# bempt/uda_aerial_semantic_segmentation_research

Hardware: AMD Instinct MI355X
Metric: training images/sec at 512x512 (higher is better)
Workload: dtype fp32

## Files before the change

### include/udaseg.h

```cpp
#ifndef UDASEG_H
#define UDASEG_H

#include <stddef.h>
#include <stdint.h>

#ifdef __cplusplus
extern "C" {
#endif

#define UDASEG_OK 0
#define UDASEG_E_BADARG (-1)
#define UDASEG_E_UNSUPPORTED (-2)
#define UDASEG_E_WORKSPACE (-3)
#define UDASEG_E_HIP (-4)

#define UDASEG_ACT_NONE 0
#define UDASEG_ACT_LEAKY 1

int udaseg_version(void);
#define UDASEG_OPT_GENERIC_GATHER 0
#define UDASEG_OPT_F32_SPLIT 1
#define UDASEG_OPT_WGRAD_GENERIC 2
#define UDASEG_OPT_F32_HALO 3
#define UDASEG_OPT_F3_CFG 4
// ... 5 lines not shown
#define UDASEG_OPT_WGRAD_X3_BLOCKS 10
#define UDASEG_OPT_WGRAD_BLOCKS 11
#define UDASEG_OPT_WGRAD_NO_XCD 12
#define UDASEG_OPT_WGRAD_X3 13
#define UDASEG_OPT_NO_WGRAD_HALO 14
#define UDASEG_OPT_WGRAD_F3_BLOCKS 15
#define UDASEG_OPT_WGRAD_HALO_BLOCKS 16
#define UDASEG_OPT_WGRAD_DEEP_BLOCKS 17
#define UDASEG_OPT_WGRAD_DB 18
#define UDASEG_OPT_REDUCE_BLOCKS 19
#define UDASEG_OPT_BN_APPLY_PT 20
#define UDASEG_OPT_GEMM_1X1_TILE 21
#define UDASEG_OPT_GEMM_1X1 22
#define UDASEG_OPT_GEMM_1X1_MAXM 23
#define UDASEG_OPT_NO_STREAM 24
#define UDASEG_OPT_HALO_CFG 25
#define UDASEG_OPT_NO_HALO 26
#define UDASEG_OPT_NO_HALO_S2 27
#define UDASEG_OPT_HALO_W16 28
#define UDASEG_OPT_HALO_DEEP 29
#define UDASEG_OPT_HALO_S2_CK 30
#define UDASEG_OPT_UP_CFG 31
#define UDASEG_OPT_WGRAD_UP_BLOCKS 32
#define UDASEG_OPT_COUNT 33
int udaseg_set_option(int key, int value);
int udaseg_get_option(int key);
int udaseg_option_count(void);
const char* udaseg_option_name(int key);
int udaseg_option_epoch(void);
const char* udaseg_last_error(void);
int udaseg_device_count(void);
int udaseg_memset_async(void* ptr, int value, size_t bytes, void* stream);
int udaseg_stream_wait(void* waiter_stream, void* signal_stream);

typedef struct {
  int n, hi, wi, ci;
  int ho, wo, co;
  int kh, kw, stride, pad;
} udaseg_conv_desc;


int udaseg_conv2d_fwd(const udaseg_conv_desc* d, const float* x, const float* w, const float* bias, float* y,
                      int act, float slope, int accumulate, void* stream);
int udaseg_conv2d_fwd_bnstats(const udaseg_conv_desc* d, const float* x, const float* w, const float* bias, float* y,
                              double* stats, void* stream);
int udaseg_conv2d_fwd_fused(const udaseg_conv_desc* d, const float* x, const float* w, const float* bias,
                            const float* residual, float* y, int act, float slope, void* stream);
// ... 328 lines not shown
```

### uda_aerial_semantic_segmentation_research_amd/_lib.py

```python
import ctypes as C
import os

_HERE = os.path.dirname(os.path.abspath(__file__))
LIB_PATH = os.environ.get("UDASEG_LIB", os.path.join(_HERE, "libudaseg_hip.so"))

ACT_NONE = 0
ACT_LEAKY = 1


class ConvDesc(C.Structure):
    _fields_ = [(k, C.c_int) for k in ("n", "hi", "wi", "ci", "ho", "wo", "co", "kh", "kw", "stride", "pad")]


_P = C.c_void_p
_I = C.c_int
_L = C.c_int64
_F = C.c_float
_D = C.POINTER(ConvDesc)

SIGNATURES = {
    "udaseg_version": (_I, []),
    "udaseg_set_option": (_I, [_I, _I]),
    "udaseg_get_option": (_I, [_I]),
    "udaseg_option_count": (_I, []),
# ... 145 lines not shown
    "udaseg_conv2d_wgrad_up_f32x3": (_I, [_D, _P, _I, _P, _P, _P]),
    "udaseg_conv2d_wgrad_halo_slice_f32x3": (_I, [_D, _P, _P, _P, _I, _I, _P]),
    "udaseg_wgrad_up_set_blocks": (_I, [_I]),
    "udaseg_conv_stem_f32x3_ok": (_I, [_D]),
    "udaseg_conv2d_fwd_stem_f32x3": (_I, [_D, _P, _P, _P, _P, _P]),
    "udaseg_conv_n16_f32x3_ok": (_I, [_D, _I]),
    "udaseg_conv2d_fwd_n16_f32x3": (_I, [_D, _P, _P, _P, _I, _F, _P, _P, _P, _P]),
    "udaseg_conv2d_dgrad_n16_f32x3": (_I, [_D, _P, _P, _P, _P, _P, _P, _P, _P, _I, _F, _P, _P]),
    "udaseg_set_workspace": (_I, [_P, C.c_size_t]),
    "udaseg_workspace_bytes": (C.c_size_t, [_D]),
    "udaseg_debug_set_timeline": (_I, [_P, _I]),
    "udaseg_fill_f32": (_I, [_P, _L, _F, _P]),
    "udaseg_axpy_f32": (_I, [_P, _P, _L, _F, _P]),
    "udaseg_add_i64": (_I, [_P, _L, _L, _P]),
    "udaseg_prof_enable": (_I, [_I]),
    "udaseg_prof_reset": (_I, []),
    "udaseg_prof_read": (_I, [_I, C.POINTER(C.c_double), C.POINTER(C.c_double), C.POINTER(C.c_int64)]),
    "udaseg_prof_kernel_count": (_I, []),
    "udaseg_prof_kernel_name": (C.c_char_p, [_I]),
    "udaseg_prof_kernel_read": (_I, [_I, C.POINTER(C.c_double), C.POINTER(C.c_double), C.POINTER(C.c_int64)]),
    "udaseg_prof_records": (_I, [_I, _I, C.POINTER(C.c_double), C.POINTER(C.c_double), C.POINTER(C.c_int), C.POINTER(C.c_int)]),
}

OPTIONS = {"GENERIC_GATHER": 0, "F32_SPLIT": 1, "WGRAD_GENERIC": 2, "F32_HALO": 3, "F3_CFG": 4, "F3_WS": 5, "F3_SIGNS": 6, "IGEMM_TILE": 7, "IGEMM_X3": 8, "NO_FOLD": 9, "WGRAD_X3_BLOCKS": 10, "WGRAD_BLOCKS": 11, "WGRAD_NO_XCD": 12, "WGRAD_X3": 13, "NO_WGRAD_HALO": 14, "WGRAD_F3_BLOCKS": 15, "WGRAD_HALO_BLOCKS": 16, "WGRAD_DEEP_BLOCKS": 17, "WGRAD_DB": 18, "REDUCE_BLOCKS": 19, "BN_APPLY_PT": 20, "GEMM_1X1_TILE": 21, "GEMM_1X1": 22, "GEMM_1X1_MAXM": 23, "NO_STREAM": 24, "HALO_CFG": 25, "NO_HALO": 26, "NO_HALO_S2": 27, "HALO_W16": 28, "HALO_DEEP": 29, "HALO_S2_CK": 30, "UP_CFG": 31, "WGRAD_UP_BLOCKS": 32}

_lib = None


def load():
    global _lib
    if _lib is not None:
        return _lib
    if not os.path.exists(LIB_PATH):
        raise RuntimeError(
            f"{LIB_PATH} not found: the HIP extension is not built. Run `python -c \"import __graft_entry__ as g; "
            f"g.build()\"` (or `make -C {os.path.join(_HERE, 'csrc')}`). There is no CPU fallback.")
    lib = C.CDLL(LIB_PATH)
    for name, (res, args) in SIGNATURES.items():
        fn = getattr(lib, name)
        fn.restype = res
        fn.argtypes = args
    _lib = lib
    return lib


def check(rc, what=""):
    if rc != 0:
# ... 10 lines not shown
```

### uda_aerial_semantic_segmentation_research_amd/csrc/api.hip

```cpp
#include <string.h>
#include <mutex>
#include <vector>

#include "common.h"
#include "options.h"

namespace udaseg {

static thread_local char g_err[512] = "";

void set_error(const char* fmt, ...) {
  va_list ap;
  va_start(ap, fmt);
  vsnprintf(g_err, sizeof(g_err), fmt, ap);
  va_end(ap);
}

int hip_fail(hipError_t e, const char* what) {
  set_error("%s: %s", what, hipGetErrorString(e));
  return UDASEG_E_HIP;
}

struct ProfRec {
  hipEvent_t a, b;
// ... 221 lines not shown
     {"UDASEG_NO_FOLD", K_FLAG, 0},
     {"UDASEG_WGRAD_X3_BLOCKS", K_INT, 1024},
     {"UDASEG_WGRAD_BLOCKS", K_INT, 0},
     {"UDASEG_WGRAD_NO_XCD", K_FLAG, 0},
     {"UDASEG_WGRAD_X3", K_OFF0, 1},
     {"UDASEG_NO_WGRAD_HALO", K_FLAG, 0},
     {"UDASEG_WGRAD_F3_BLOCKS", K_INT, 120},
     {"UDASEG_WGRAD_HALO_BLOCKS", K_INT, 96},
     {"UDASEG_WGRAD_DEEP_BLOCKS", K_INT, 0},
     {"UDASEG_WGRAD_DB", K_INT, 1},
     {"UDASEG_REDUCE_BLOCKS", K_INT, 0},
     {"UDASEG_BN_APPLY_PT", K_INT, 4},
     {"UDASEG_GEMM_1X1_TILE", K_INT, 0},
     {"UDASEG_GEMM_1X1", K_OFF0, 1},
     {"UDASEG_GEMM_1X1_MAXM", K_INT, 73728},
     {"UDASEG_NO_STREAM", K_FLAG, 0},
     {"UDASEG_HALO_CFG", K_INT, 0},
     {"UDASEG_NO_HALO", K_FLAG, 0},
     {"UDASEG_NO_HALO_S2", K_FLAG, 0},
     {"UDASEG_HALO_W16", K_INT, 6},
     {"UDASEG_HALO_DEEP", K_OFF0, 1},
     {"UDASEG_HALO_S2_CK", K_INT, 64},
     {"UDASEG_UP_CFG", K_INT, 0},
     {"UDASEG_WGRAD_UP_BLOCKS", K_INT, 0}};
int g_opt_val[UDASEG_OPT_COUNT];
static int g_opt_default[UDASEG_OPT_COUNT];
std::atomic<bool> g_opt_ready{false};
static std::atomic<int> g_opt_epoch{0};
static std::mutex g_opt_mutex;
void opt_init() {
  std::lock_guard<std::mutex> lk(g_opt_mutex);
  if (g_opt_ready.load(std::memory_order_relaxed)) return;
  for (int k = 0; k < UDASEG_OPT_COUNT; ++k) {
    const OptRow& r = g_opt_rows[k];
    const char* e = getenv(r.env);
    int v = r.dflt;
    if (r.kind == K_INT) v = e ? atoi(e) : r.dflt;
    else if (r.kind == K_FLAG) v = e != nullptr ? 1 : 0;
    else v = (e && atoi(e) == 0) ? 0 : 1;
    g_opt_default[k] = g_opt_val[k] = v;
  }
  g_opt_ready.store(true, std::memory_order_release);
}
}

extern "C" int udaseg_set_option(int key, int value) {
  UDASEG_CHECK_ARG(key >= 0 && key < UDASEG_OPT_COUNT, "set_option: unknown key %d (0 .. %d)", key, UDASEG_OPT_COUNT - 1);
// ... 40 lines not shown
```

### uda_aerial_semantic_segmentation_research_amd/csrc/conv_wgrad.hip

```cpp
#include <stdlib.h>

#include <type_traits>

#include "common.h"
#include "halo_common.h"

namespace udaseg {

struct WgradArgs {
  const void* x;
  const void* dy;
  float* dw;
  int hi, wi, ci, ho, wo, co;
  int kw, stride, pad;
  int M, J;
  int kchunk;
  int use_atomic;
  float inv_ci, inv_kw, inv_wo, inv_ho;
  int row_uniform;
  unsigned x_bytes, dy_bytes;
  int ci_full, c_off, J_ld, up;
  const float* in_scale;
  const float* in_shift;
  int in_act;
// ... 953 lines not shown
  return f32 ? (off || !f32_halo_enabled()) : off;
}
}

extern "C" int udaseg_conv2d_wgrad_bnin_ok(const udaseg_conv_desc* d, int up) {
  if (!d || d->kh != 3 || d->kw != 3 || d->stride != 1 || d->pad != 1 || d->n <= 0 || d->hi <= 0 || d->wi <= 0 || d->ci % 8 != 0 ||
      d->co % 4 != 0)
    return 0;
  if (small_wgrad_applicable(d->kh, d->stride, d->pad, d->ci, d->co, d->n * cdiv(d->hi, 16) * cdiv(d->wi, 16))) return 1;
  return !up && !wgrad_halo_off(true) && wgrad_h2_applicable(d, 0, true) ? 1 : 0;
}

extern "C" int udaseg_conv2d_wgrad_bnin(const udaseg_conv_desc* d, const float* x, int up, const float* in_scale, const float* in_shift,
                                        int in_act, float in_slope, const float* dy, float* dw, int accumulate, void* stream) {
  UDASEG_CHECK_ARG(d && x && in_scale && in_shift && dy && dw, "conv2d_wgrad_bnin: NULL pointer");
  UDASEG_CHECK_ARG(in_act == UDASEG_ACT_NONE || in_act == UDASEG_ACT_LEAKY, "conv2d_wgrad_bnin: unknown activation %d", in_act);
  UDASEG_CHECK_ARG(d->ho == d->hi && d->wo == d->wi, "conv2d_wgrad_bnin: stride-1 'same' convolutions only");
  UDASEG_CHECK_ARG(!up || (d->hi % 2 == 0 && d->wi % 2 == 0), "conv2d_wgrad_bnin: an up-sampled source needs even extents");
  if (!udaseg_conv2d_wgrad_bnin_ok(d, up)) {
    set_error("conv2d_wgrad_bnin: geometry not supported (ask udaseg_conv2d_wgrad_bnin_ok)");
    return UDASEG_E_UNSUPPORTED;
  }
  hipStream_t st = as_stream(stream);
  const bool small = small_wgrad_applicable(d->kh, d->stride, d->pad, d->ci, d->co, d->n * cdiv(d->hi, 16) * cdiv(d->wi, 16));
  if (!small && !accumulate) {
    hipError_t e = hipMemsetAsync(dw, 0, (size_t)d->co * 9 * d->ci * sizeof(float), st);
    if (e != hipSuccess) return hip_fail(e, "hipMemsetAsync(dw)");
  }
  prof_begin(1, st);
  int rc;
  if (small) {
    rc = launch_small_wgrad(x, dy, dw, d->n, d->hi, d->wi, d->ci, d->co, accumulate, st, up, in_scale, in_shift, in_act, in_slope);
  } else {
    rc = launch_wgrad_h2(d, x, nullptr, 0, dy, dw, true, st, in_scale, in_shift, in_act, in_slope);
  }
  prof_end(1, st, udaseg_conv_flops(d), 2, d);
  return rc;
}

extern "C" int udaseg_conv2d_wgrad_halo_bf16_ok(const udaseg_conv_desc* d, int up_ca) {
  return d != nullptr && !wgrad_halo_off(false) && wgrad_h2_applicable(d, up_ca, false) ? 1 : 0;
}

extern "C" int udaseg_conv2d_wgrad_halo_bf16(const udaseg_conv_desc* d, const void* x, const void* skip, int up_ca, const void* dy,
                                             float* dw, void* stream) {
  UDASEG_CHECK_ARG(d && x && dy && dw, "conv2d_wgrad_halo_bf16: NULL pointer");
  UDASEG_CHECK_ARG(d->n > 0 && d->hi > 0 && d->wi > 0 && d->ho == d->hi && d->wo == d->wi, "conv2d_wgrad_halo_bf16: bad extents");
  UDASEG_CHECK_ARG(up_ca == 0 ? skip == nullptr : skip != nullptr, "conv2d_wgrad_halo_bf16: up_ca and skip come together");
  if (!udaseg_conv2d_wgrad_halo_bf16_ok(d, up_ca)) {
    set_error("conv2d_wgrad_halo_bf16: geometry not supported (ask udaseg_conv2d_wgrad_halo_bf16_ok first)");
    return UDASEG_E_UNSUPPORTED;
  }
  hipStream_t st = as_stream(stream);
  prof_begin(1, st);
  const int rc = launch_wgrad_h2(d, x, skip, up_ca, dy, dw, false, st);
  prof_end(1, st, udaseg_conv_flops(d), 2, d);
  return rc;
}

extern "C" int udaseg_conv2d_wgrad_halo_f32x3_ok(const udaseg_conv_desc* d, int up_ca) {
  return d != nullptr && !wgrad_halo_off(true) && wgrad_h2_applicable(d, up_ca, true) ? 1 : 0;
}

extern "C" int udaseg_conv2d_wgrad_halo_f32x3(const udaseg_conv_desc* d, const float* x, const float* skip, int up_ca, const float* dy,
                                              float* dw, void* stream) {
  UDASEG_CHECK_ARG(d && x && dy && dw, "conv2d_wgrad_halo_f32x3: NULL pointer");
  UDASEG_CHECK_ARG(d->n > 0 && d->hi > 0 && d->wi > 0 && d->ho == d->hi && d->wo == d->wi, "conv2d_wgrad_halo_f32x3: bad extents");
  UDASEG_CHECK_ARG((up_ca > 0) == (skip != nullptr), "conv2d_wgrad_halo_f32x3: up_ca=%d, skip %s", up_ca, skip ? "given" : "NULL");
  if (!udaseg_conv2d_wgrad_halo_f32x3_ok(d, up_ca)) {
    set_error("conv2d_wgrad_halo_f32x3: geometry not supported (ask udaseg_conv2d_wgrad_halo_f32x3_ok first)");
    return UDASEG_E_UNSUPPORTED;
  }
  hipStream_t st = as_stream(stream);
  prof_begin(1, st);
  const int rc = launch_wgrad_h2(d, x, skip, up_ca, dy, dw, true, st);
  prof_end(1, st, udaseg_conv_flops(d), 2, d);
  return rc;
}

extern "C" int udaseg_conv2d_wgrad_halo_slice_f32x3(const udaseg_conv_desc* d, const float* x, const float* dy, float* dw, int ldw,
                                                    int c_off, void* stream) {
  UDASEG_CHECK_ARG(d && x && dy && dw, "conv2d_wgrad_halo_slice_f32x3: NULL pointer");
  UDASEG_CHECK_ARG(d->n > 0 && d->hi > 0 && d->wi > 0 && d->ho == d->hi && d->wo == d->wi, "conv2d_wgrad_halo_slice_f32x3: bad extents");
  UDASEG_CHECK_ARG(ldw >= d->ci && c_off >= 0 && c_off + d->ci <= ldw && c_off % 4 == 0 && ldw % 4 == 0,
                   "conv2d_wgrad_halo_slice_f32x3: slice [%d, %d) of rows of %d channels", c_off, c_off + d->ci, ldw);
  if (!udaseg_conv2d_wgrad_halo_f32x3_ok(d, 0)) {
    set_error("conv2d_wgrad_halo_slice_f32x3: geometry not supported (ask udaseg_conv2d_wgrad_halo_f32x3_ok on the slice's descriptor)");
    return UDASEG_E_UNSUPPORTED;
  }
  hipStream_t st = as_stream(stream);
  prof_begin(1, st);
// ... 68 lines not shown
```

### uda_aerial_semantic_segmentation_research_amd/csrc/conv_wgrad_halo2.hip

```cpp
#include <stdlib.h>

#include <type_traits>

#include "common.h"
#include "halo_common.h"

namespace udaseg {

typedef short h2_s16x4 __attribute__((ext_vector_type(4)));
typedef short h2_s16x8 __attribute__((ext_vector_type(8)));

struct WgradH2Args {
  const void* x;
  const void* x2;
  const void* dy;
  float* dw;
  int ldw, dw_coff;
  int n, h, w, ci, co, up_ca;
  int ntx, nty, ntiles, ncib, pairs, P;
  unsigned x_bytes, x2_bytes, dy_bytes;
  const float* in_scale;
  const float* in_shift;
  int in_act;
  float in_slope;
// ... 261 lines not shown
  }
  const int ci_g = cib * C::CIB + ciq * 32 + lr;
#pragma unroll
  for (int dy = 0; dy < 3; ++dy)
#pragma unroll
    for (int dxi = 0; dxi < NDX; ++dxi)
#pragma unroll
      for (int v = 0; v < 16; ++v) {
        const int co_g = cob * C::COB + coq * 32 + (v & 3) + 8 * (v >> 2) + 4 * lh;
        atomicAdd(a.dw + ((size_t)co_g * 9 + dy * 3 + DX0 + dxi) * a.ldw + a.dw_coff + ci_g, acc[dy * NDX + dxi][v]);
      }
}

template <int PL, int COQ, int CIQ, int TR, int TWK, int NSTW, bool DB, bool TL = false, bool XF = false>
__global__ __launch_bounds__(512, 2) void conv_wgrad_h2_kernel(const WgradH2Args a) {
  using C = H2<PL, COQ, CIQ, TR, TWK, NSTW, DB>;
  extern __shared__ __attribute__((aligned(16))) char h2smem[];
  const int tid = threadIdx.x, lane = tid & 63;
  const int wave = __builtin_amdgcn_readfirstlane(tid >> 6);
  if (wave < 4) wgrad_h2_role<C, 0, 2, NSTW == 8, TL, XF>(a, h2smem, tid, lane, wave);
  else wgrad_h2_role<C, 2, 1, true, TL, XF>(a, h2smem, tid, lane, wave);
}

static int h2_config(const udaseg_conv_desc* d, int up_ca, bool f32) {
  if (d->kh != 3 || d->kw != 3 || d->stride != 1 || d->pad != 1) return 0;
  if (d->n <= 0 || d->hi <= 0 || d->wi <= 0 || d->ho != d->hi || d->wo != d->wi || d->ci <= 0 || d->co <= 0) return 0;
  const long long px = (long long)d->n * d->hi * d->wi;
  const int es = f32 ? 4 : 2;
  if (px * d->ci * es >= (1LL << 31) || px * d->co * es >= (1LL << 31)) return 0;
  int cfg = 0;
  if (d->ci % 64 == 0 && d->co % 64 == 0) cfg = d->wi < 32 ? 2 : 1;
  else if (d->ci % 64 == 0 && d->co % 32 == 0) cfg = 3;
  else if (d->ci % 32 == 0 && d->co % 32 == 0) cfg = 4;
  if (cfg == 0 || d->wi < 16) return 0;
  if (cfg != 2 && d->wi < 32) return 0;
  if (up_ca > 0) {
    if (up_ca >= d->ci || d->hi % 2 != 0 || d->wi % 2 != 0) return 0;
    if (up_ca % 64 != 0) {
      if (up_ca % 32 != 0 || d->wi < 32) return 0;
      cfg = 4;
    }
  }
  return cfg;
}

bool wgrad_h2_applicable(const udaseg_conv_desc* d, int up_ca, bool f32) { return d != nullptr && h2_config(d, up_ca, f32) != 0; }

struct H2In {
  const float* scale = nullptr;
  const float* shift = nullptr;
  int act = 0;
  float slope = 0.f;
// ... 56 lines not shown
      if (!xf_attr) {
        hipError_t e = hipFuncSetAttribute(reinterpret_cast<const void*>(kern_xf), hipFuncAttributeMaxDynamicSharedMemorySize, C::LDS);
        if (e != hipSuccess) return hip_fail(e, "hipFuncSetAttribute(conv_wgrad_h2, in-staging transform)");
        xf_attr = true;
      }
      static std::atomic<int> kid_xf{-1};
      if (kid_xf < 0) {
        char nm[112];
        snprintf(nm, sizeof(nm), "conv_wgrad_h2_kernel<%d, %d, %d, %d, %d, %d, %s, false, true>", PL, COQ, CIQ, TR, TWK, NSTW, DB ? "true" : "false");
        kid_xf = kprof_id(nm);
      }
      hipLaunchKernelGGL(kern_xf, dim3((unsigned)(a.pairs * P)), dim3(C::NT), C::LDS, s, a);
      kprof_end(kid_xf, ev, s, 2.0 * (double)px * d->co * 9.0 * d->ci);
      UDASEG_LAUNCH_CHECK("conv_wgrad_h2 (in-staging transform) launch");
      return UDASEG_OK;
    }
  }
  hipLaunchKernelGGL(kern, dim3((unsigned)(a.pairs * P)), dim3(C::NT), C::LDS, s, a);
  kprof_end(kid, ev, s, 2.0 * (double)px * d->co * 9.0 * d->ci);
  UDASEG_LAUNCH_CHECK("conv_wgrad_h2 launch");
  return UDASEG_OK;
}

int launch_wgrad_h2(const udaseg_conv_desc* d, const void* x, const void* x2, int up_ca, const void* dy, float* dw, bool f32,
                    hipStream_t s, const float* in_scale, const float* in_shift, int in_act, float in_slope, int ldw, int dw_coff) {
  H2In in;
  in.scale = in_scale; in.shift = in_shift; in.act = in_act; in.slope = in_slope;
  in.ldw = ldw; in.dw_coff = dw_coff;
  if (in_scale != nullptr && (!f32 || up_ca != 0 || in_shift == nullptr)) {
    set_error("conv2d_wgrad_halo: the in-staging transform needs fp32 operands and a single plain source");
    return UDASEG_E_UNSUPPORTED;
  }
  const int cfg = h2_config(d, up_ca, f32);
  if (cfg == 0) {
    set_error("conv2d_wgrad_halo: geometry not supported (ask the _ok query first)");
    return UDASEG_E_UNSUPPORTED;
  }
  int tf3 = opt_get(UDASEG_OPT_WGRAD_F3_BLOCKS), tbf = opt_get(UDASEG_OPT_WGRAD_HALO_BLOCKS);
  const int tdeep_o = opt_get(UDASEG_OPT_WGRAD_DEEP_BLOCKS);
  const int tdeep = tdeep_o >= 1 ? tdeep_o : 256;
  const int tdeep3 = tdeep_o >= 1 ? tdeep_o : 128;
  if (tf3 < 1) tf3 = 120;
  if (tbf < 1) tbf = 96;
  const int db = opt_get(UDASEG_OPT_WGRAD_DB);
  if (f32) {
    if (cfg == 1 && db) return launch_h2_t<3, 2, 2, 2, 2, 4, true>(d, x, x2, up_ca, dy, dw, s, tf3, in);
    if (cfg == 1) return launch_h2_t<3, 2, 2, 4, 2, 4>(d, x, x2, up_ca, dy, dw, s, tf3, in);
    if (cfg == 2) return launch_h2_t<3, 2, 2, 8, 1, 4>(d, x, x2, up_ca, dy, dw, s, tdeep3, in);
    if (cfg == 3) return launch_h2_t<3, 1, 2, 4, 2, 4>(d, x, x2, up_ca, dy, dw, s, tf3, in);
    return launch_h2_t<3, 1, 1, 4, 2, 4>(d, x, x2, up_ca, dy, dw, s, tf3, in);
  }
  if (cfg == 1) return launch_h2_t<1, 2, 2, 8, 2, 8>(d, x, x2, up_ca, dy, dw, s, tbf);
  if (cfg == 2) return launch_h2_t<1, 2, 2, 8, 1, 8>(d, x, x2, up_ca, dy, dw, s, tdeep);
  if (cfg == 3) return launch_h2_t<1, 1, 2, 8, 2, 8>(d, x, x2, up_ca, dy, dw, s, tbf);
  return launch_h2_t<1, 1, 1, 8, 2, 8>(d, x, x2, up_ca, dy, dw, s, tbf);
}

struct WgradUpArgs {
  const float* x;
  const float* dy;
  float* dw;
  int n, h, w, ca, co, ldw;
  int ntx, nty, ntiles, ncib, pairs, P;
  unsigned x_bytes, dy_bytes;
};

template <int COQ_, int CIQ_, int TR_, int TWK_>
struct H2Up {
// ... 269 lines not shown
```

### uda_aerial_semantic_segmentation_research_amd/engine.py

```python
import math
import os
import weakref

import torch
import torch.nn as nn

from . import kernels as K
from ._lib import ACT_LEAKY, ACT_NONE

ALIGN = 64
SIDE_STREAM_WGRAD = os.environ.get("UDASEG_SERIAL", "0") != "1"
FUSE_BN_REDUCE = os.environ.get("UDASEG_FUSE_BN_REDUCE", "1") != "0"
PREPACK_DGRAD = os.environ.get("UDASEG_PREPACK", "2") in ("1", "2")
PREPACK_ALL = os.environ.get("UDASEG_PREPACK", "2") == "2"
USE_FRAG_KERNELS = os.environ.get("UDASEG_FRAG", "1") != "0"
FRAG_POLICY = "always" if os.environ.get("UDASEG_FRAG") == "2" else "auto"
USE_F32_SPLIT = os.environ.get("UDASEG_F32_SPLIT", "1") != "0"
USE_UP_PHASE = os.environ.get("UDASEG_UP_PHASE", "1") != "0"
USE_N16 = os.environ.get("UDASEG_N16", "1") != "0"
USE_STEM = os.environ.get("UDASEG_STEM", "1") != "0"
PRELAUNCH_SKIP = os.environ.get("UDASEG_PRELAUNCH_SKIP", "1") != "0"


FUSE_BN_APPLY = os.environ.get("UDASEG_FUSE_BN_APPLY", "0") != "0"
# ... 726 lines not shown
            K.pack_dgrad_batched(net._arena, net._wt_arena, net._wt_table, self.st)
        if self.frag and net._frag_bwd_table is not None and not self._packed_all:
            K.pack_frag_batched(None, net._wt_arena, net._frag_arena, net._frag_bwd_table, self.st)
        if self.frag and net._up_bwd_table is not None and not self._packed_all:
            K.pack_up_batched(None, net._wt_arena, net._frag_arena, net._up_bwd_table, self.st)
        if self.side_stream is not None:
            self.side_stream.wait_stream(self.main_stream)

    def packed_wt(self, conv):
        o = self.net._wt_off[id(conv)]
        n = conv.cout_p * conv.k * conv.k * conv.cin_p
        return self.net._wt_arena[o:o + n]

    def _next_bstats(self, c):
        o = self._bstat_off
        self._bstat_off += 2 * c
        return self.bstats[o * self.R:(o + 2 * c) * self.R]

    def wgrad_route(self, d, x):
        up = isinstance(x, UpCat)
        if isinstance(x.a if up else x, LazyAct):
            return BNIN
        if up:
            both = self._wgrad_halo and x.skip is not None and K.conv2d_wgrad_halo_ok(d, x.a.shape[-1], f32=not self.bf16)
            return HALO if both else PART
        return HALO if self._wgrad_halo and K.conv2d_wgrad_halo_ok(d, f32=not self.bf16) else GENERIC

    def dgrad_route(self, conv, d, x, dx, dx_acc):
        if isinstance(dx, UpGrad):
            return PHASE, self.up_frag(conv, d, x.a.shape[-1])
        n16 = self.n16_frag(conv, d, True) if not (dx_acc or isinstance(x, UpCat)) else None
        if n16 is not None:
            return N16, n16
        wfd = self.wfrag(conv, d, dgrad=True)
        if isinstance(x, UpCat):
            if wfd is not None and (x.skip is None or x.a.shape[-1] % 32 == 0):
                return FRAG, wfd
            return (IGEMM if x.skip is None else SPLIT), None
        return (FRAG, wfd) if wfd is not None else (IGEMM, None)

    def _bn_reduce_by(self, prev):
        bs = self._bnb[id(prev.y)] = self._next_bstats(prev.y.shape[-1] if self.bf16 else ceil4(prev.bn.c))
        return prev.bn_reduce_args(self, bs)

    def conv_bwd(self, conv, d, x, dy, dx=None, dx_acc=False, dbias=None, prev=None):
        side = self.side_stream
        if side is not None:
# ... 125 lines not shown
```

Before: 1025.

## Add pair-packed fp32x3 halo wgrad kernels for narrow 16-channel convs

Adds new halo weight-gradient kernel variants for 3x3 convs with 16 input channels (and an upsampled 32-channel no-skip form). They pack channel pairs, use bf16x3-split MFMA with double-buffered LDS, split K across waves, and reduce through LDS before atomic adds. Narrow-channel layers and upsampled layers without a skip now take this route instead of the small or generic wgrad kernels, replacing an inefficient path for low-channel layers. The trade-offs are more atomics and new numerical paths, including a sign-flipping accumulation trick.

```diff
diff --git a/include/udaseg.h b/include/udaseg.h
--- a/include/udaseg.h
+++ b/include/udaseg.h
@@ -51,7 +51,9 @@
 #define UDASEG_OPT_HALO_S2_CK 30
 #define UDASEG_OPT_UP_CFG 31
 #define UDASEG_OPT_WGRAD_UP_BLOCKS 32
-#define UDASEG_OPT_COUNT 33
+#define UDASEG_OPT_WGRAD_PAIR 33
+#define UDASEG_OPT_WGRAD_PAIR_BLOCKS 34
+#define UDASEG_OPT_COUNT 35
 int udaseg_set_option(int key, int value);
 int udaseg_get_option(int key);
 int udaseg_option_count(void);
diff --git a/uda_aerial_semantic_segmentation_research_amd/_lib.py b/uda_aerial_semantic_segmentation_research_amd/_lib.py
--- a/uda_aerial_semantic_segmentation_research_amd/_lib.py
+++ b/uda_aerial_semantic_segmentation_research_amd/_lib.py
@@ -191,7 +191,7 @@
     "udaseg_prof_records": (_I, [_I, _I, C.POINTER(C.c_double), C.POINTER(C.c_double), C.POINTER(C.c_int), C.POINTER(C.c_int)]),
 }
 
-OPTIONS = {"GENERIC_GATHER": 0, "F32_SPLIT": 1, "WGRAD_GENERIC": 2, "F32_HALO": 3, "F3_CFG": 4, "F3_WS": 5, "F3_SIGNS": 6, "IGEMM_TILE": 7, "IGEMM_X3": 8, "NO_FOLD": 9, "WGRAD_X3_BLOCKS": 10, "WGRAD_BLOCKS": 11, "WGRAD_NO_XCD": 12, "WGRAD_X3": 13, "NO_WGRAD_HALO": 14, "WGRAD_F3_BLOCKS": 15, "WGRAD_HALO_BLOCKS": 16, "WGRAD_DEEP_BLOCKS": 17, "WGRAD_DB": 18, "REDUCE_BLOCKS": 19, "BN_APPLY_PT": 20, "GEMM_1X1_TILE": 21, "GEMM_1X1": 22, "GEMM_1X1_MAXM": 23, "NO_STREAM": 24, "HALO_CFG": 25, "NO_HALO": 26, "NO_HALO_S2": 27, "HALO_W16": 28, "HALO_DEEP": 29, "HALO_S2_CK": 30, "UP_CFG": 31, "WGRAD_UP_BLOCKS": 32}
+OPTIONS = {"GENERIC_GATHER": 0, "F32_SPLIT": 1, "WGRAD_GENERIC": 2, "F32_HALO": 3, "F3_CFG": 4, "F3_WS": 5, "F3_SIGNS": 6, "IGEMM_TILE": 7, "IGEMM_X3": 8, "NO_FOLD": 9, "WGRAD_X3_BLOCKS": 10, "WGRAD_BLOCKS": 11, "WGRAD_NO_XCD": 12, "WGRAD_X3": 13, "NO_WGRAD_HALO": 14, "WGRAD_F3_BLOCKS": 15, "WGRAD_HALO_BLOCKS": 16, "WGRAD_DEEP_BLOCKS": 17, "WGRAD_DB": 18, "REDUCE_BLOCKS": 19, "BN_APPLY_PT": 20, "GEMM_1X1_TILE": 21, "GEMM_1X1": 22, "GEMM_1X1_MAXM": 23, "NO_STREAM": 24, "HALO_CFG": 25, "NO_HALO": 26, "NO_HALO_S2": 27, "HALO_W16": 28, "HALO_DEEP": 29, "HALO_S2_CK": 30, "UP_CFG": 31, "WGRAD_UP_BLOCKS": 32, "WGRAD_PAIR": 33, "WGRAD_PAIR_BLOCKS": 34}
 
 _lib = None
 
diff --git a/uda_aerial_semantic_segmentation_research_amd/csrc/api.hip b/uda_aerial_semantic_segmentation_research_amd/csrc/api.hip
--- a/uda_aerial_semantic_segmentation_research_amd/csrc/api.hip
+++ b/uda_aerial_semantic_segmentation_research_amd/csrc/api.hip
@@ -267,7 +267,9 @@
      {"UDASEG_HALO_DEEP", K_OFF0, 1},
      {"UDASEG_HALO_S2_CK", K_INT, 64},
      {"UDASEG_UP_CFG", K_INT, 0},
-     {"UDASEG_WGRAD_UP_BLOCKS", K_INT, 0}};
+     {"UDASEG_WGRAD_UP_BLOCKS", K_INT, 0},
+     {"UDASEG_WGRAD_PAIR", K_INT, 4},
+     {"UDASEG_WGRAD_PAIR_BLOCKS", K_INT, 0}};
 int g_opt_val[UDASEG_OPT_COUNT];
 static int g_opt_default[UDASEG_OPT_COUNT];
 std::atomic<bool> g_opt_ready{false};
diff --git a/uda_aerial_semantic_segmentation_research_amd/csrc/conv_wgrad.hip b/uda_aerial_semantic_segmentation_research_amd/csrc/conv_wgrad.hip
--- a/uda_aerial_semantic_segmentation_research_amd/csrc/conv_wgrad.hip
+++ b/uda_aerial_semantic_segmentation_research_amd/csrc/conv_wgrad.hip
@@ -999,7 +999,8 @@
     return UDASEG_E_UNSUPPORTED;
   }
   hipStream_t st = as_stream(stream);
-  const bool small = small_wgrad_applicable(d->kh, d->stride, d->pad, d->ci, d->co, d->n * cdiv(d->hi, 16) * cdiv(d->wi, 16));
+  const bool pair = !up && d->ci <= 16 && !wgrad_halo_off(true) && wgrad_h2_applicable(d, 0, true);
+  const bool small = !pair && small_wgrad_applicable(d->kh, d->stride, d->pad, d->ci, d->co, d->n * cdiv(d->hi, 16) * cdiv(d->wi, 16));
   if (!small && !accumulate) {
     hipError_t e = hipMemsetAsync(dw, 0, (size_t)d->co * 9 * d->ci * sizeof(float), st);
     if (e != hipSuccess) return hip_fail(e, "hipMemsetAsync(dw)");
@@ -1043,7 +1044,7 @@
                                               float* dw, void* stream) {
   UDASEG_CHECK_ARG(d && x && dy && dw, "conv2d_wgrad_halo_f32x3: NULL pointer");
   UDASEG_CHECK_ARG(d->n > 0 && d->hi > 0 && d->wi > 0 && d->ho == d->hi && d->wo == d->wi, "conv2d_wgrad_halo_f32x3: bad extents");
-  UDASEG_CHECK_ARG((up_ca > 0) == (skip != nullptr), "conv2d_wgrad_halo_f32x3: up_ca=%d, skip %s", up_ca, skip ? "given" : "NULL");
+  UDASEG_CHECK_ARG((up_ca > 0 && up_ca < d->ci) == (skip != nullptr), "conv2d_wgrad_halo_f32x3: up_ca=%d, skip %s", up_ca, skip ? "given" : "NULL");
   if (!udaseg_conv2d_wgrad_halo_f32x3_ok(d, up_ca)) {
     set_error("conv2d_wgrad_halo_f32x3: geometry not supported (ask udaseg_conv2d_wgrad_halo_f32x3_ok first)");
     return UDASEG_E_UNSUPPORTED;
diff --git a/uda_aerial_semantic_segmentation_research_amd/csrc/conv_wgrad_halo2.hip b/uda_aerial_semantic_segmentation_research_amd/csrc/conv_wgrad_halo2.hip
--- a/uda_aerial_semantic_segmentation_research_amd/csrc/conv_wgrad_halo2.hip
+++ b/uda_aerial_semantic_segmentation_research_amd/csrc/conv_wgrad_halo2.hip
@@ -307,12 +307,402 @@
   else wgrad_h2_role<C, 2, 1, true, TL, XF>(a, h2smem, tid, lane, wave);
 }
 
+template <int TR_, int TWK_>
+struct H2P {
+  static constexpr int PL = 3, TR = TR_, TWK = TWK_;
+  static constexpr bool UP = false;
+  static constexpr int NT = 512;
+  static constexpr int TW = 32 * TWK, HR = TR + 2, HWD = TW + 2, HP = HR * HWD, TP = TR * TW;
+  static constexpr int KS = 4;
+  static constexpr int KSH = KS < TWK ? KS : TWK, KSR = KS / KSH;
+  static constexpr int RW = TR / KSR, NHF = TWK / KSH;
+  static constexpr int XPLANE = HP * 32, DPLANE = TP * 32;
+  static constexpr int BUF = PL * (XPLANE + DPLANE);
+  static constexpr int LDS = 2 * BUF;
+  static constexpr int XPC = HP * 2, DPC = TP * 2;
+  static constexpr int NX = (XPC + NT - 1) / NT, ND = (DPC + NT - 1) / NT;
+  static_assert(TR % KSR == 0 && TWK % KSH == 0 && KSH * KSR == KS, "K split tiles the tile");
+  static_assert(LDS <= 160 * 1024 && 6 * 24 * 64 * 4 <= LDS, "LDS");
+};
+
+template <typename C, bool XF>
+__device__ __forceinline__ void wgrad_h2p_role(const WgradH2Args& a, char* smem, int tid, int lane, int wave) {
+  constexpr int PL = 3;
+  char* const Xs = smem;
+  char* const Ds = smem + PL * C::XPLANE;
+  const int lr = lane & 31, lh = lane >> 5;
+  const int grp = lane >> 4, cb = 16 * (grp & 1), hk = grp >> 1, tq = (lane & 15) >> 2, tp = lane & 3;
+  const int sg = wave & 1, ks = wave >> 1;
+  const int ksh = ks % C::KSH, r0 = (ks / C::KSH) * C::RW;
+  const int cob = (int)blockIdx.x % a.pairs, split = (int)blockIdx.x / a.pairs;
+  const int H = a.h, W = a.w;
+  __amdgpu_buffer_rsrc_t rs_x = __builtin_amdgcn_make_buffer_rsrc(const_cast<void*>(a.x), 0, (int)a.x_bytes, 0x00020000);
+  __amdgpu_buffer_rsrc_t rs_d = __builtin_amdgcn_make_buffer_rsrc(const_cast<void*>(a.dy), 0, (int)a.dy_bytes, 0x00020000);
+  u32x4 sx[C::NX][2], sd[C::ND][2];
+  unsigned x_in = 0;
+  f32x4 xsc[2] = {{0.f, 0.f, 0.f, 0.f}, {0.f, 0.f, 0.f, 0.f}}, xsh[2] = {{0.f, 0.f, 0.f, 0.f}, {0.f, 0.f, 0.f, 0.f}};
+  if constexpr (XF) {
+    const int ch = (tid & 1) * 8;
+    xsc[0] = *reinterpret_cast<const f32x4*>(a.in_scale + ch);
+    xsc[1] = *reinterpret_cast<const f32x4*>(a.in_scale + ch + 4);
+    xsh[0] = *reinterpret_cast<const f32x4*>(a.in_shift + ch);
+    xsh[1] = *reinterpret_cast<const f32x4*>(a.in_shift + ch + 4);
+  }
+  const int dch = cob * 16 + (tid & 1) * 8;
+  auto load_tile = [&](int tile) {
+    x_in = 0;
+    const int tx = tile % a.ntx;
+    const int t2 = tile / a.ntx;
+    const int ty = t2 % a.nty, img = t2 / a.nty;
+    const int y0 = ty * C::TR, x0 = tx * C::TW;
+#pragma unroll
+    for (int i = 0; i < C::NX; ++i) {
+      const int pc = tid + i * C::NT;
+      const int pix = pc >> 1, oct = pc & 1;
+      const int hy = pix / C::HWD, hx = pix - hy * C::HWD;
+      const int iy = y0 + hy - 1, ix = x0 + hx - 1;
+      const bool ok = pc < C::XPC && (unsigned)iy < (unsigned)H && (unsigned)ix < (unsigned)W;
+      const unsigned off = ok ? (unsigned)((((img * H + iy) * W + ix) * 16 + oct * 8) * 4) : 0x80000000u;
+      if constexpr (XF) x_in |= (ok ? 1u : 0u) << i;
+#pragma unroll
+      for (int l = 0; l < 2; ++l) sx[i][l] = __builtin_amdgcn_raw_buffer_load_b128(rs_x, (int)off, 16 * l, 0);
+    }
+#pragma unroll
+    for (int i = 0; i < C::ND; ++i) {
+      const int pc = tid + i * C::NT;
+      const int pix = pc >> 1;
+      const int oy = y0 + pix / C::TW, ox = x0 + pix % C::TW;
+      const bool ok = pc < C::DPC && oy < H && ox < W && dch < a.co;
+      const unsigned off = ok ? (unsigned)((((img * H + oy) * W + ox) * a.co + dch) * 4) : 0x80000000u;
+#pragma unroll
+      for (int l = 0; l < 2; ++l) sd[i][l] = __builtin_amdgcn_raw_buffer_load_b128(rs_d, (int)off, 16 * l, 0);
+    }
+  };
+  auto store_piece = [&](char* dst, int plane_bytes, const u32x4 (&v)[2], unsigned sgn) {
+    u32x4 p0, p1, p2;
+    split3(v[0] ^ sgn, v[1] ^ sgn, p0, p1, p2);
+    *reinterpret_cast<u32x4*>(dst) = p0;
+    *reinterpret_cast<u32x4*>(dst + plane_bytes) = p1;
+    *reinterpret_cast<u32x4*>(dst + 2 * plane_bytes) = p2;
+  };
+  const int nseq = split < a.ntiles ? (a.ntiles - split + a.P - 1) / a.P : 0;
+  const int sq1 = (nseq + 2) / 4, sq3 = nseq - sq1;
+  auto store_tile = [&](int bo, int seq) {
+    const unsigned dsgn = (seq >= sq1 && seq < sq3) ? 0x80000000u : 0u;
+#pragma unroll
+    for (int i = 0; i < C::NX; ++i) {
+      const int pc = tid + i * C::NT;
+      if constexpr (XF) {
+        const bool in = (x_in >> i) & 1u;
+#pragma unroll
+        for (int l = 0; l < 2; ++l) {
+          f32x4 v = __builtin_bit_cast(f32x4, sx[i][l]);
+#pragma unroll
+          for (int e = 0; e < 4; ++e) {
+            const float t = act_apply(__builtin_fmaf(v[e], xsc[l][e], xsh[l][e]), a.in_act, a.in_slope);
+            v[e] = in ? t : 0.f;
+          }
+          sx[i][l] = __builtin_bit_cast(u32x4, v);
+        }
+      }
+      if (i < C::NX - 1 || pc < C::XPC) store_piece(Xs + bo + pc * 16, C::XPLANE, sx[i], 0u);
+    }
+#pragma unroll
+    for (int i = 0; i < C::ND; ++i) {
+      const int pc = tid + i * C::NT;
+      if (i < C::ND - 1 || pc < C::DPC) store_piece(Ds + bo + pc * 16, C::DPLANE, sd[i], dsgn);
+    }
+  };
+
+  f32x16 acc[3];
+#pragma unroll
+  for (int t = 0; t < 3; ++t)
+#pragma unroll
+    for (int v = 0; v < 16; ++v) acc[t][v] = 0.f;
+
+  const int lane_off = (8 * hk + tq) * 64 + (cb + 4 * tp) * 2;
+  const char* const dbase0 = Ds + (r0 * C::TW + 32 * ksh) * 32 + lane_off;
+  const char* const xbase0 = Xs + (r0 * C::HWD + 32 * ksh + 2 * sg) * 32 + lane_off;
+
+  int cur = 0;
+  if (split < a.ntiles) load_tile(split);
+  store_tile(0, 0);
+  if (split + a.P < a.ntiles) load_tile(split + a.P);
+  __syncthreads();
+  int seq = 0;
+  bool negated = false;
+  for (int tile = split; tile < a.ntiles; tile += a.P, ++seq) {
+    if ((seq >= sq1 && seq < sq3) != negated) {
+      negated = !negated;
+#pragma unroll
+      for (int t = 0; t < 3; ++t) acc[t] = -acc[t];
+    }
+    if (tile + a.P < a.ntiles) {
+      store_tile(cur ^ C::BUF, seq + 1);
+      if (tile + 2 * a.P < a.ntiles) load_tile(tile + 2 * a.P);
+    }
+    const char* const dbase = dbase0 + cur;
+    const char* const xbase = xbase0 + cur;
+    cur ^= C::BUF;
+#pragma unroll
+    for (int hfi = 0; hfi < C::NHF; ++hfi) {
+      bf16x8 A[3][PL];
+#pragma unroll
+      for (int rr = 0; rr < C::RW + 2; ++rr) {
+        if (rr < C::RW) {
+#pragma unroll
+          for (int pl = 0; pl < PL; ++pl)
+            A[rr % 3][pl] = h2_tr_fragment(dbase + pl * C::DPLANE + (rr * C::TW + 32 * C::KSH * hfi) * 32);
+        }
+        bf16x8 B[PL];
+#pragma unroll
+        for (int pl = 0; pl < PL; ++pl) B[pl] = h2_tr_fragment(xbase + pl * C::XPLANE + (rr * C::HWD + 32 * C::KSH * hfi) * 32);
+#pragma unroll
+        for (int ky = 0; ky < 3; ++ky) {
+          const int j = rr - ky;
+          if (j >= 0 && j < C::RW) {
+#pragma unroll
+            for (int ij = 2; ij >= 0; --ij)
+#pragma unroll
+              for (int i = 0; i <= ij; ++i)
+                acc[ky] = __builtin_amdgcn_mfma_f32_32x32x16_bf16(A[j % 3][i], B[ij - i], acc[ky], 0, 0, 0);
+          }
+        }
+      }
+    }
+    __syncthreads();
+  }
+  if (negated) {
+#pragma unroll
+    for (int t = 0; t < 3; ++t) acc[t] = -acc[t];
+  }
+  const bool lo = lr < 16;
+  float out[24];
+#pragma unroll
+  for (int ky = 0; ky < 3; ++ky)
+#pragma unroll
+    for (int v = 0; v < 8; ++v) {
+      const float other = __shfl_xor(acc[ky][v + 8], 16);
+      out[ky * 8 + v] = lo ? acc[ky][v] + other : (sg ? other : acc[ky][v]);
+    }
+  float* const red = reinterpret_cast<float*>(smem);
+  if (ks != 0) {
+#pragma unroll
+    for (int j = 0; j < 24; ++j) red[(((ks - 1) * 2 + sg) * 24 + j) * 64 + lane] = out[j];
+  }
+  __syncthreads();
+  if (ks != 0) return;
+#pragma unroll
+  for (int k2 = 0; k2 < 3; ++k2)
+#pragma unroll
+    for (int j = 0; j < 24; ++j) out[j] += red[((k2 * 2 + sg) * 24 + j) * 64 + lane];
+  const int ci_g = lr & 15;
+  const int kx = lo ? 2 * sg : 1;
+#pragma unroll
+  for (int ky = 0; ky < 3; ++ky)
+#pragma unroll
+    for (int v = 0; v < 8; ++v) {
+      const int co_g = cob * 16 + (v & 3) + 8 * (v >> 2) + 4 * lh;
+      if (co_g < a.co) atomicAdd(a.dw + ((size_t)co_g * 9 + ky * 3 + kx) * a.ldw + a.dw_coff + ci_g, out[ky * 8 + v]);
+    }
+}
+
+template <int TR_, int TWK_>
+struct H2PU {
+  static constexpr int PL = 3, TR = TR_, TWK = TWK_;
+  static constexpr bool UP = true;
+  static constexpr int NT = 512;
+  static constexpr int TW = 32 * TWK, AR = TR / 2 + 2, AW = TW / 2 + 2, AP = AR * AW, TP = TR * TW;
+  static constexpr int XPLANE = AP * 64, DPLANE = TP * 32;
+  static constexpr int BUF = PL * (XPLANE + DPLANE);
+  static constexpr int LDS = 2 * BUF;
+  static constexpr int XPC = AP * 4, DPC = TP * 2;
+  static constexpr int NX = (XPC + NT - 1) / NT, ND = (DPC + NT - 1) / NT;
+  static_assert(TR % 2 == 0 && (TR / 2) * TWK == 4, "one (row, half) of each parity per wave");
+  static_assert(LDS <= 160 * 1024 && 6 * 48 * 64 * 4 <= LDS, "LDS");
+};
+
+template <typename C>
+__device__ __forceinline__ void wgrad_h2pu_role(const WgradH2Args& a, char* smem, int tid, int lane, int wave) {
+  constexpr int PL = 3;
+  char* const Xs = smem;
+  char* const Ds = smem + PL * C::XPLANE;
+  const int lr = lane & 31, lh = lane >> 5;
+  const int grp = lane >> 4, cb = 16 * (grp & 1), hk = grp >> 1, tq = (lane & 15) >> 2, tp = lane & 3;
+  const int py = wave & 1, ks = wave >> 1;
+  const int ksh = ks % C::TWK, rsel = ks / C::TWK;
+  const int split = (int)blockIdx.x;
+  const int H = a.h, W = a.w, HA = a.h >> 1, WA = a.w >> 1;
+  __amdgpu_buffer_rsrc_t rs_x = __builtin_amdgcn_make_buffer_rsrc(const_cast<void*>(a.x), 0, (int)a.x_bytes, 0x00020000);
+  __amdgpu_buffer_rsrc_t rs_d = __builtin_amdgcn_make_buffer_rsrc(const_cast<void*>(a.dy), 0, (int)a.dy_bytes, 0x00020000);
+  u32x4 sx[C::NX][2], sd[C::ND][2];
+  auto load_tile = [&](int tile) {
+    const int tx = tile % a.ntx;
+    const int t2 = tile / a.ntx;
+    const int ty = t2 % a.nty, img = t2 / a.nty;
+    const int y0 = ty * C::TR, x0 = tx * C::TW;
+#pragma unroll
+    for (int i = 0; i < C::NX; ++i) {
+      const int pc = tid + i * C::NT;
+      const int pix = pc >> 2, oct = pc & 3;
+      const int hy = pix / C::AW, hx = pix - hy * C::AW;
+      const int iy = (y0 >> 1) + hy - 1, ix = (x0 >> 1) + hx - 1;
+      const bool ok = pc < C::XPC && (unsigned)iy < (unsigned)HA && (unsigned)ix < (unsigned)WA;
+      const unsigned off = ok ? (unsigned)((((img * HA + iy) * WA + ix) * 32 + oct * 8) * 4) : 0x80000000u;
+#pragma unroll
+      for (int l = 0; l < 2; ++l) sx[i][l] = __builtin_amdgcn_raw_buffer_load_b128(rs_x, (int)off, 16 * l, 0);
+    }
+#pragma unroll
+    for (int i = 0; i < C::ND; ++i) {
+      const int pc = tid + i * C::NT;
+      const int pix = pc >> 1, oct = pc & 1;
+      const int oy = y0 + pix / C::TW, ox = x0 + pix % C::TW;
+      const bool ok = pc < C::DPC && oy < H && ox < W;
+      const unsigned off = ok ? (unsigned)((((img * H + oy) * W + ox) * 16 + oct * 8) * 4) : 0x80000000u;
+#pragma unroll
+      for (int l = 0; l < 2; ++l) sd[i][l] = __builtin_amdgcn_raw_buffer_load_b128(rs_d, (int)off, 16 * l, 0);
+    }
+  };
+  auto store_piece = [&](char* dst, int plane_bytes, const u32x4 (&v)[2], unsigned sgn) {
+    u32x4 p0, p1, p2;
+    split3(v[0] ^ sgn, v[1] ^ sgn, p0, p1, p2);
+    *reinterpret_cast<u32x4*>(dst) = p0;
+    *reinterpret_cast<u32x4*>(dst + plane_bytes) = p1;
+    *reinterpret_cast<u32x4*>(dst + 2 * plane_bytes) = p2;
+  };
+  const int nseq = split < a.ntiles ? (a.ntiles - split + a.P - 1) / a.P : 0;
+  const int sq1 = (nseq + 2) / 4, sq3 = nseq - sq1;
+  auto store_tile = [&](int bo, int seq) {
+    const unsigned dsgn = (seq >= sq1 && seq < sq3) ? 0x80000000u : 0u;
+#pragma unroll
+    for (int i = 0; i < C::NX; ++i) {
+      const int pc = tid + i * C::NT;
+      if (i < C::NX - 1 || pc < C::XPC) store_piece(Xs + bo + pc * 16, C::XPLANE, sx[i], 0u);
+    }
+#pragma unroll
+    for (int i = 0; i < C::ND; ++i) {
+      const int pc = tid + i * C::NT;
+      if (i < C::ND - 1 || pc < C::DPC) store_piece(Ds + bo + pc * 16, C::DPLANE, sd[i], dsgn);
+    }
+  };
+
+  f32x16 acc[6];
+#pragma unroll
+  for (int t = 0; t < 6; ++t)
+#pragma unroll
+    for (int v = 0; v < 16; ++v) acc[t][v] = 0.f;
+
+  const int lane_off = (8 * hk + tq) * 64 + (cb + 4 * tp) * 2;
+  const char* const dbase0 = Ds + ((2 * rsel + py) * C::TW + 32 * ksh) * 32 + lane_off;
+  const char* const xbase0 = Xs + ((rsel + py) * C::AW + 16 * ksh) * 64 + lane_off;
+
+  int cur = 0;
+  if (split < a.ntiles) load_tile(split);
+  store_tile(0, 0);
+  if (split + a.P < a.ntiles) load_tile(split + a.P);
+  __syncthreads();
+  int seq = 0;
+  bool negated = false;
+  for (int tile = split; tile < a.ntiles; tile += a.P, ++seq) {
+    if ((seq >= sq1 && seq < sq3) != negated) {
+      negated = !negated;
+#pragma unroll
+      for (int t = 0; t < 6; ++t) acc[t] = -acc[t];
+    }
+    if (tile + a.P < a.ntiles) {
+      store_tile(cur ^ C::BUF, seq + 1);
+      if (tile + 2 * a.P < a.ntiles) load_tile(tile + 2 * a.P);
+    }
+    const char* const dbase = dbase0 + cur;
+    const char* const xbase = xbase0 + cur;
+    cur ^= C::BUF;
+    bf16x8 A[PL];
+#pragma unroll
+    for (int pl = 0; pl < PL; ++pl) A[pl] = h2_tr_fragment(dbase + pl * C::DPLANE);
+#pragma unroll
+    for (int u = 0; u < 2; ++u)
+#pragma unroll
+      for (int e = 0; e < 3; ++e) {
+        bf16x8 B[PL];
+#pragma unroll
+        for (int pl = 0; pl < PL; ++pl) B[pl] = h2_tr_fragment(xbase + pl * C::XPLANE + (u * C::AW + e) * 64);
+#pragma unroll
+        for (int ij = 2; ij >= 0; --ij)
+#pragma unroll
+          for (int i = 0; i <= ij; ++i)
+            acc[u * 3 + e] = __builtin_amdgcn_mfma_f32_32x32x16_bf16(A[i], B[ij - i], acc[u * 3 + e], 0, 0, 0);
+      }
+    __syncthreads();
+  }
+  if (negated) {
+#pragma unroll
+    for (int t = 0; t < 6; ++t) acc[t] = -acc[t];
+  }
+  float out[48];
+#pragma unroll
+  for (int u = 0; u < 2; ++u)
+#pragma unroll
+    for (int v = 0; v < 8; ++v) {
+      out[(u * 3 + 0) * 8 + v] = acc[u * 3 + 0][v] + acc[u * 3 + 1][v + 8];
+      out[(u * 3 + 1) * 8 + v] = acc[u * 3 + 1][v] + acc[u * 3 + 1][v + 8];
+      out[(u * 3 + 2) * 8 + v] = acc[u * 3 + 1][v] + acc[u * 3 + 2][v + 8];
+    }
+  float* const red = reinterpret_cast<float*>(smem);
+  if (ks != 0) {
+#pragma unroll
+    for (int j = 0; j < 48; ++j) red[(((ks - 1) * 2 + py) * 48 + j) * 64 + lane] = out[j];
+  }
+  __syncthreads();
+  if (ks != 0) return;
+#pragma unroll
+  for (int k2 = 0; k2 < 3; ++k2)
+#pragma unroll
+    for (int j = 0; j < 48; ++j) out[j] += red[((k2 * 2 + py) * 48 + j) * 64 + lane];
+  auto emit = [&](int u, int ky) {
+#pragma unroll
+    for (int v = 0; v < 8; ++v) {
+      const int co_g = (v & 3) + 8 * (v >> 2) + 4 * lh;
+      float* const row = a.dw + ((size_t)co_g * 9 + ky * 3) * a.ldw + a.dw_coff + lr;
+#pragma unroll
+      for (int kx = 0; kx < 3; ++kx) atomicAdd(row + kx * a.ldw, out[(u * 3 + kx) * 8 + v]);
+    }
+  };
+  if (py == 0) {
+    emit(0, 0); emit(1, 1); emit(1, 2);
+  } else {
+    emit(0, 0); emit(0, 1); emit(1, 2);
+  }
+}
+
+template <int PL, typename C, bool XF>
+__global__ __launch_bounds__(512, 1) void conv_wgrad_h2_kernel(const WgradH2Args a) {
+  static_assert(PL == 3, "the pair-packed form is fp32 split only");
+  extern __shared__ __attribute__((aligned(16))) char h2smem[];
+  const int tid = threadIdx.x, lane = tid & 63;
+  const int wave = __builtin_amdgcn_readfirstlane(tid >> 6);
+  if constexpr (C::UP) wgrad_h2pu_role<C>(a, h2smem, tid, lane, wave);
+  else wgrad_h2p_role<C, XF>(a, h2smem, tid, lane, wave);
+}
+
+static bool h2_pair_up_config(const udaseg_conv_desc* d, int up_ca, bool f32) {
+  if (!f32 || up_ca != 32 || d->ci != 32 || d->co != 16) return false;
+  if (d->hi % 2 != 0 || d->wi % 2 != 0 || d->wi < 16) return false;
+  return (opt_get(UDASEG_OPT_WGRAD_PAIR) & 4) != 0;
+}
+static bool h2_pair_config(const udaseg_conv_desc* d, int up_ca, bool f32) {
+  if (!f32 || up_ca != 0 || d->ci != 16 || d->co < 8 || d->co > 32 || d->co % 8 != 0) return false;
+  if (d->wi % 2 != 0 || d->wi < 16) return false;
+  return (opt_get(UDASEG_OPT_WGRAD_PAIR) & (d->co <= 16 ? 1 : 2)) != 0;
+}
+
 static int h2_config(const udaseg_conv_desc* d, int up_ca, bool f32) {
   if (d->kh != 3 || d->kw != 3 || d->stride != 1 || d->pad != 1) return 0;
   if (d->n <= 0 || d->hi <= 0 || d->wi <= 0 || d->ho != d->hi || d->wo != d->wi || d->ci <= 0 || d->co <= 0) return 0;
   const long long px = (long long)d->n * d->hi * d->wi;
   const int es = f32 ? 4 : 2;
   if (px * d->ci * es >= (1LL << 31) || px * d->co * es >= (1LL << 31)) return 0;
+  if (h2_pair_config(d, up_ca, f32)) return 5;
+  if (h2_pair_up_config(d, up_ca, f32)) return 6;
   int cfg = 0;
   if (d->ci % 64 == 0 && d->co % 64 == 0) cfg = d->wi < 32 ? 2 : 1;
   else if (d->ci % 64 == 0 && d->co % 32 == 0) cfg = 3;
@@ -415,6 +805,50 @@
   return UDASEG_OK;
 }
 
+template <typename C>
+static int launch_h2p_t(const udaseg_conv_desc* d, const void* x, const void* dy, float* dw, hipStream_t s, int target, const H2In& in) {
+  WgradH2Args a = {};
+  a.x = x; a.dy = dy; a.dw = dw;
+  a.ldw = in.ldw > 0 ? in.ldw : d->ci; a.dw_coff = in.ldw > 0 ? in.dw_coff : 0;
+  a.in_scale = in.scale; a.in_shift = in.shift; a.in_act = in.act; a.in_slope = in.slope;
+  a.n = d->n; a.h = d->hi; a.w = d->wi; a.ci = d->ci; a.co = d->co;
+  a.ntx = cdiv(d->wi, C::TW); a.nty = cdiv(d->hi, C::TR); a.ntiles = d->n * a.ntx * a.nty;
+  a.ncib = 1; a.pairs = cdiv(d->co, 16);
+  int P = target / a.pairs;
+  if (P < 1) P = 1;
+  if (P > a.ntiles) P = a.ntiles;
+  a.P = P;
+  const long long px = (long long)d->n * d->hi * d->wi;
+  a.x_bytes = (unsigned)((C::UP ? px / 4 : px) * d->ci * 4);
+  a.dy_bytes = (unsigned)(px * d->co * 4);
+  if (C::UP && a.in_scale != nullptr) {
+    set_error("conv2d_wgrad_halo: the pair-packed up-sampled form takes a written source only");
+    return UDASEG_E_UNSUPPORTED;
+  }
+  const bool xf = a.in_scale != nullptr;
+  auto kern = conv_wgrad_h2_kernel<3, C, false>;
+  if constexpr (!C::UP) {
+    if (xf) kern = conv_wgrad_h2_kernel<3, C, true>;
+  }
+  static std::atomic<bool> attr_done[2] = {};
+  if (!attr_done[xf]) {
+    hipError_t e = hipFuncSetAttribute(reinterpret_cast<const void*>(kern), hipFuncAttributeMaxDynamicSharedMemorySize, C::LDS);
+    if (e != hipSuccess) return hip_fail(e, "hipFuncSetAttribute(conv_wgrad_h2, pair-packed)");
+    attr_done[xf] = true;
+  }
+  static std::atomic<int> kid[2] = {{-1}, {-1}};
+  if (kid[xf] < 0) {
+    char nm[96];
+    snprintf(nm, sizeof(nm), "conv_wgrad_h2_kernel<3, udaseg::H2P%s<%d, %d>, %s>", C::UP ? "U" : "", C::TR, C::TWK, xf ? "true" : "false");
+    kid[xf] = kprof_id(nm);
+  }
+  hipEvent_t ev = kprof_begin(s);
+  hipLaunchKernelGGL(kern, dim3((unsigned)(a.pairs * P)), dim3(C::NT), C::LDS, s, a);
+  kprof_end(kid[xf], ev, s, 2.0 * (double)px * d->co * 9.0 * d->ci);
+  UDASEG_LAUNCH_CHECK("conv_wgrad_h2 (pair-packed) launch");
+  return UDASEG_OK;
+}
+
 int launch_wgrad_h2(const udaseg_conv_desc* d, const void* x, const void* x2, int up_ca, const void* dy, float* dw, bool f32,
                     hipStream_t s, const float* in_scale, const float* in_shift, int in_act, float in_slope, int ldw, int dw_coff) {
   H2In in;
@@ -437,6 +871,14 @@
   if (tbf < 1) tbf = 96;
   const int db = opt_get(UDASEG_OPT_WGRAD_DB);
   if (f32) {
+    if (cfg == 5) {
+      const int tp = opt_get(UDASEG_OPT_WGRAD_PAIR_BLOCKS);
+      return launch_h2p_t<H2P<4, 2>>(d, x, dy, dw, s, tp >= 1 ? tp : 120, in);
+    }
+    if (cfg == 6) {
+      const int tp = opt_get(UDASEG_OPT_WGRAD_PAIR_BLOCKS);
+      return launch_h2p_t<H2PU<4, 2>>(d, x, dy, dw, s, tp >= 1 ? tp : 120, in);
+    }
     if (cfg == 1 && db) return launch_h2_t<3, 2, 2, 2, 2, 4, true>(d, x, x2, up_ca, dy, dw, s, tf3, in);
     if (cfg == 1) return launch_h2_t<3, 2, 2, 4, 2, 4>(d, x, x2, up_ca, dy, dw, s, tf3, in);
     if (cfg == 2) return launch_h2_t<3, 2, 2, 8, 1, 4>(d, x, x2, up_ca, dy, dw, s, tdeep3, in);
diff --git a/uda_aerial_semantic_segmentation_research_amd/engine.py b/uda_aerial_semantic_segmentation_research_amd/engine.py
--- a/uda_aerial_semantic_segmentation_research_amd/engine.py
+++ b/uda_aerial_semantic_segmentation_research_amd/engine.py
@@ -772,7 +772,7 @@
         if isinstance(x.a if up else x, LazyAct):
             return BNIN
         if up:
-            both = self._wgrad_halo and x.skip is not None and K.conv2d_wgrad_halo_ok(d, x.a.shape[-1], f32=not self.bf16)
+            both = self._wgrad_halo and K.conv2d_wgrad_halo_ok(d, x.a.shape[-1], f32=not self.bf16)
             return HALO if both else PART
         return HALO if self._wgrad_halo and K.conv2d_wgrad_halo_ok(d, f32=not self.bf16) else GENERIC
 
```

Result: faster. 1036, median of 6 (+1.1%).
